# Zeudon/sound-event-localization-detection

Hardware: AMD Instinct MI355X
Metric: training clips/sec (4ch FOA 60s@24kHz) (higher is better)
Workload: dtype bf16; 1 GPU; crnn FOA 4-ch 60s clips, bs=32 windows (BASELINE configs[1]); parallelism=dp1

## Files before the change

include/seld_hip.h:

```cpp
#ifndef SELD_HIP_H_
#define SELD_HIP_H_

#include <stdint.h>

#ifdef __cplusplus
extern "C" {
#endif

int seld_init(int device);
int seld_shutdown(void);
int seld_version(void);
const char* seld_last_error(void);

int seld_set_mel_filterbank(const float* fb_host);

int seld_set_window(const float* window_host);

int seld_default_tables(float* window960, float* fb481x64, int* mel_b0_64, float* mel_wd_24x64,
                        float* mel_wu_24x64);

int64_t seld_num_frames(int64_t L);

int seld_logmel_f32(const float* pcm, int64_t N, int64_t C, int64_t L, float* out, int layout, void* stream);
int seld_logmel_i16(const int16_t* pcm, int64_t N, int64_t C, int64_t L, float* out, int layout, void* stream);
// ... 107 lines not shown
int seld_convfirst_forward(const void* in, const void* w, int w_is_bf16, int64_t w_sco, int64_t w_sci, int64_t w_sr,
                           int64_t w_ss, int64_t B, int64_t T, int64_t F, const float* bn_weight, const float* bn_bias,
                           float* running_mean, float* running_var, float momentum, float eps, void* y,
                           float* mean_invstd, float* scale_shift, float* workspace, int phases, void* stream);
int seld_convfirst_backward(const void* in, const void* w, int w_is_bf16, int64_t w_sco, int64_t w_sci, int64_t w_sr,
                            int64_t w_ss, const void* dy, int64_t B, int64_t T, int64_t F, const float* mean_invstd,
                            const float* scale_shift, void* dw, int dw_is_bf16, int64_t dw_sco, int64_t dw_sci,
                            int64_t dw_sr, int64_t dw_ss, float* dgamma, float* dbeta, float* workspace, int phases,
                            void* stream);

int64_t seld_conv_tail_workspace_floats(int C);
int seld_conv_tail_forward(const void* x, const void* residual, int is_bf16, int64_t rows, int C, int pool,
                           const float* weight, const float* bias, float* running_mean, float* running_var,
                           float momentum, float eps, int training, void* y, float* mean_invstd, float* scale_shift,
                           float* workspace, void* stream);
int seld_conv_tail_backward(const void* x, const void* residual, const void* dy, int is_bf16, int64_t rows, int C,
                            int pool, const float* mean_invstd, const float* scale_shift, void* dx, void* dresidual,
                            float* dweight, float* dbias, float* workspace, void* stream);

int seld_dwconv1d(const void* x, int is_bf16, const float* weight, const float* bias, int64_t B, int64_t T, int D, int K,
                  int flip_taps, void* y, void* stream);
int64_t seld_dwconv1d_wgrad_rows(int64_t B, int64_t T);
int seld_dwconv1d_wgrad(const void* x, const void* dy, int is_bf16, int64_t B, int64_t T, int D, int K, float* partial,
                        void* stream);

int64_t seld_gru_tile_rows(void);
int seld_gru_forward(const void* gi, int is_bf16, const void* w_hh_bf16, const float* b_hn, int64_t B,
                     int64_t T, int64_t H, void* y, void* saved_tile, void* stream);

int seld_gru_backward(const void* dy_tile, const void* saved_tile, const void* y, int is_bf16,
                      const void* w_hh_t_bf16, int64_t tiles, int64_t T, int64_t H, void* dg_tile, float* dbias,
                      void* stream);

int seld_gru_to_tile(const void* src, int elem_bytes, int64_t B, int64_t T, int ns, void* dst, void* stream);
int seld_gru_from_pair_tile(const void* dg_tile, int elem_bytes, int64_t B, int64_t T, void* dgi, void* dghn,
                            void* stream);

int seld_gru_previous_state(const void* y, int elem_bytes, int64_t B, int64_t T, void* h_prev, void* stream);

int seld_grid_decode(const void* logits, int is_bf16, int64_t w0, int64_t nw, int64_t W, int64_t total,
                     const int64_t* meta_first, const int32_t* meta_len, int64_t q0, int64_t nq, float threshold, int K,
                     int32_t* det_cell, float* det_score, int32_t* det_count, float* probs_out, void* stream);

int seld_doa_match(const int32_t* det_cell, const int32_t* det_count, int K, const int32_t* ref_offsets,
                   const int32_t* ref_dirs, int64_t nq, int I, int J, double thr_deg, int32_t* stats, double* cost,
                   void* stream);

#ifdef __cplusplus
}
#endif
#endif
```

sound-event-localization-detection_amd/csrc/gru.hip:

```cpp
#include <hip/hip_bf16.h>
#include <stdlib.h>

#include "seld_common.h"

#ifndef SELD_GRU_SEQS
#define SELD_GRU_SEQS 4
#endif

namespace seld {

constexpr int kH = 256;
constexpr int kG = 3 * kH;
constexpr int kRows = 16;
constexpr int kSeqs = SELD_GRU_SEQS;
constexpr int kParts = kRows / kSeqs;
constexpr int kU = 8 / kParts;
constexpr int kGruThreads = 512;
constexpr int kHPitch = kH + 8;
constexpr int kDghPitch = kG + 8;
constexpr int kWnBytes = 8 * 2 * 8 * 64 * 16;
static_assert(kSeqs == 8 || kSeqs == 4, "8 or 4 sequences per tile");

typedef __attribute__((ext_vector_type(8))) __bf16 bf16x8;
typedef __attribute__((ext_vector_type(4))) float f32x4;

__device__ __forceinline__ float sigmoid_f(float x) { return __builtin_amdgcn_rcpf(1.0f + __expf(-x)); }
__device__ __forceinline__ float tanh_f(float x) { return fmaf(-2.0f, __builtin_amdgcn_rcpf(1.0f + __expf(2.0f * x)), 1.0f); }

template <int kPart> __device__ __forceinline__ float shifted_part(float old, float src) {
  constexpr int ctrl = 0x110 + kPart * kSeqs;
  constexpr int banks = kSeqs == 8 ? 0xc : (1 << kPart);
  return __int_as_float(__builtin_amdgcn_update_dpp(__float_as_int(old), __float_as_int(src), ctrl, 0xf, banks, false));
}
__device__ __forceinline__ void own_values(const f32x4 (&v)[2], float (&out)[kU]) {
#pragma unroll
  for (int j = 0; j < kU; ++j) {
    float r = v[j >> 2][j & 3];
    if (kParts >= 2) r = shifted_part<1>(r, v[(kU + j) >> 2][(kU + j) & 3]);
    if (kParts == 4) {
      r = shifted_part<2>(r, v[(2 * kU + j) >> 2][(2 * kU + j) & 3]);
      r = shifted_part<3>(r, v[(3 * kU + j) >> 2][(3 * kU + j) & 3]);
    }
    out[j] = r;
  }
}

template <int kBytes> struct Raw;
template <> struct alignas(4) Raw<4> { unsigned w[1]; };
template <> struct alignas(8) Raw<8> { unsigned w[2]; };
template <> struct alignas(16) Raw<16> { unsigned w[4]; };
template <> struct alignas(16) Raw<32> { unsigned w[8]; };

typedef _Float16 f16x2 __attribute__((ext_vector_type(2)));
typedef float f32x2 __attribute__((ext_vector_type(2)));
__device__ __forceinline__ unsigned pack_bf16x2(float lo, float hi) {
  return static_cast<unsigned>(__bfloat16_as_ushort(__float2bfloat16(lo))) |
         (static_cast<unsigned>(__bfloat16_as_ushort(__float2bfloat16(hi))) << 16);
// ... 204 lines not shown
template <typename T>
__global__ __launch_bounds__(kGruThreads, 2) void gru_forward_kernel(GruFwdArgs a) {
  extern __shared__ __attribute__((aligned(16))) unsigned char smem[];
  bf16x8* wn_lds = reinterpret_cast<bf16x8*>(smem);
  __hip_bfloat16* hbuf = reinterpret_cast<__hip_bfloat16*>(smem + kWnBytes);
  const int tid = threadIdx.x;
  const int wave = tid >> 6, lane = tid & 63;
  const int q = lane >> 4, c = lane & 15;
  const __hip_bfloat16* w = a.w_hh + static_cast<long>(blockIdx.y) * kG * kH;

  bf16x8 wr[2][8], wz[2][8];
#pragma unroll
  for (int s = 0; s < 2; ++s) {
    const int unit = 32 * wave + 16 * s + c;
#pragma unroll
    for (int kk = 0; kk < 8; ++kk) {
      const int k0 = 32 * kk + 8 * q;
      wr[s][kk] = *reinterpret_cast<const bf16x8*>(w + static_cast<long>(unit) * kH + k0);
      wz[s][kk] = *reinterpret_cast<const bf16x8*>(w + static_cast<long>(kH + unit) * kH + k0);
      wn_lds[((wave * 2 + s) * 8 + kk) * 64 + lane] =
          *reinterpret_cast<const bf16x8*>(w + static_cast<long>(2 * kH + unit) * kH + k0);
    }
  }
  for (int i = tid; i < 2 * kSeqs * kHPitch; i += kGruThreads) hbuf[i] = __float2bfloat16(0.0f);
  __syncthreads();
  if (a.saved) gru_forward_steps<T, true>(a, wn_lds, hbuf, wr, wz);
  else gru_forward_steps<T, false>(a, wn_lds, hbuf, wr, wz);
}

struct GruBwdArgs {
  const void* dy;
  const void* saved;
  const void* y;
  const __hip_bfloat16* w_hh_t;
  void* dg;
  float* dbias;
  long tiles, T;
};

template <typename T> struct GruStepIn {
  PairOf<typename Types<T>::Saved> rz, ng;
  Group<typename Types<T>::Data> hp, d;
};

template <typename T>
__device__ __forceinline__ void gru_backward_steps(const GruBwdArgs& a, bf16x8* wn_lds, __hip_bfloat16* dgh,
                                                   const bf16x8 (&wrz)[2][16]) {
  typedef typename Types<T>::Data D;
  typedef typename Types<T>::Saved S;
  const int tid = threadIdx.x;
  const int wave = tid >> 6, lane = tid & 63;
  const int q = lane >> 4, c = lane & 15;
  const int seq = c % kSeqs;
  const int unit0 = lane_unit0(wave, lane);
  const int dir = blockIdx.y;
  const long tile = blockIdx.x;
  const Group<D>* dy = static_cast<const Group<D>*>(a.dy);
  const PairOf<S>* saved = static_cast<const PairOf<S>*>(a.saved);
  const T* y = static_cast<const T*>(a.y);
  PairOf<D>* dg = static_cast<PairOf<D>*>(a.dg);
  const long b = tile * kSeqs + seq;

  float dh[kU], bsum[4][kU];
#pragma unroll
  for (int i = 0; i < kU; ++i) {
    dh[i] = 0.0f;
#pragma unroll
    for (int k = 0; k < 4; ++k) bsum[k][i] = 0.0f;
  }

  auto time_of = [&](long step) { return dir == 0 ? step : a.T - 1 - step; };
  auto load_step = [&](long step, GruStepIn<T>& in) {
    const long tt = time_of(step);
    const long tprev = time_of(step > 0 ? step - 1 : 0);
    const PairOf<S>* sp = saved + tile_group(tile, a.T, tt, dir, wave, 2, 0, lane);
    in.rz = sp[0];
    in.ng = sp[64];
    in.hp = *reinterpret_cast<const Group<D>*>(y + (b * a.T + tprev) * (2 * kH) + dir * kH + unit0);
    in.d = dy[tile_group(tile, a.T, tt, dir, wave, 1, 0, lane)];
  };

  auto step = [&](long t, GruStepIn<T>& in) {
    const long tt = time_of(t);
    float r[kU], z[kU], n[kU], g[kU], hp[kU], d[kU];
    dec2<S>(in.rz, r, z);
    dec2<S>(in.ng, n, g);
    dec1<D>(in.hp, hp);
    dec1<D>(in.d, d);
    __builtin_amdgcn_sched_barrier(0);
    load_step(t > 1 ? t - 2 : 0, in);
    __builtin_amdgcn_sched_barrier(0);
    float keep[kU], da_r[kU], da_z[kU], da_n[kU], dghn[kU];
#pragma unroll
    for (int i = 0; i < kU; ++i) {
      const float hprev = t > 0 ? hp[i] : 0.0f;
      const float dtot = d[i] + dh[i];
      const float dn = dtot * (1.0f - z[i]);
      const float dz = dtot * (hprev - n[i]);
      da_n[i] = dn * (1.0f - n[i] * n[i]);
      da_z[i] = dz * z[i] * (1.0f - z[i]);
      da_r[i] = da_n[i] * g[i] * r[i] * (1.0f - r[i]);
      dghn[i] = da_n[i] * r[i];
      keep[i] = dtot * z[i];
      bsum[0][i] += da_r[i];
      bsum[1][i] += da_z[i];
      bsum[2][i] += da_n[i];
      bsum[3][i] += dghn[i];
    }
    PairOf<D>* const gp = dg + tile_group(tile, a.T, tt, dir, wave, 2, 0, lane);
    gp[0] = enc2<D>(da_r, da_z);
    gp[64] = enc2<D>(da_n, dghn);
    __hip_bfloat16* const dgh_cur = dgh + (t & 1) * (kSeqs * kDghPitch);
    __hip_bfloat16* drow = dgh_cur + seq * kDghPitch + unit0;
    *reinterpret_cast<Group<AsBF16>*>(drow) = enc1<AsBF16>(da_r);
    *reinterpret_cast<Group<AsBF16>*>(drow + kH) = enc1<AsBF16>(da_z);
    *reinterpret_cast<Group<AsBF16>*>(drow + 2 * kH) = enc1<AsBF16>(dghn);
    __syncthreads();

    f32x4 acc[2][2];
#pragma unroll
    for (int s = 0; s < 2; ++s)
#pragma unroll
      for (int i = 0; i < 4; ++i) acc[s][0][i] = acc[s][1][i] = 0.0f;
    const __hip_bfloat16* brow = dgh_cur + seq * kDghPitch + 8 * q;
    const bf16x8* wnp = wn_lds + wave * 2 * 8 * 64 + lane;
    bf16x8 d0 = *reinterpret_cast<const bf16x8*>(brow), d1 = *reinterpret_cast<const bf16x8*>(brow + 32);
#pragma unroll
    for (int kk = 0; kk < 24; ++kk) {
      bf16x8 d2 = d1;
      if (kk + 2 < 24) d2 = *reinterpret_cast<const bf16x8*>(brow + 32 * (kk + 2));
      if (kk < 16) {
        acc[0][kk & 1] = __builtin_amdgcn_mfma_f32_16x16x32_bf16(wrz[0][kk < 16 ? kk : 0], d0, acc[0][kk & 1], 0, 0, 0);
        acc[1][kk & 1] = __builtin_amdgcn_mfma_f32_16x16x32_bf16(wrz[1][kk < 16 ? kk : 0], d0, acc[1][kk & 1], 0, 0, 0);
      } else {
        const bf16x8 w0 = wnp[(kk - 16) * 64], w1 = wnp[(8 + kk - 16) * 64];
        acc[0][kk & 1] = __builtin_amdgcn_mfma_f32_16x16x32_bf16(w0, d0, acc[0][kk & 1], 0, 0, 0);
        acc[1][kk & 1] = __builtin_amdgcn_mfma_f32_16x16x32_bf16(w1, d0, acc[1][kk & 1], 0, 0, 0);
      }
      d0 = d1;
      d1 = d2;
    }
    f32x4 total[2];
#pragma unroll
    for (int s = 0; s < 2; ++s) total[s] = acc[s][0] + acc[s][1];
    float mine[kU];
    own_values(total, mine);
#pragma unroll
    for (int i = 0; i < kU; ++i) dh[i] = keep[i] + mine[i];
  };

  GruStepIn<T> in_a, in_b;
  load_step(a.T - 1, in_a);
  load_step(a.T > 1 ? a.T - 2 : 0, in_b);
  step(a.T - 1, in_a);
  long t = a.T - 2;
#pragma unroll 1
  for (; t >= 1; t -= 2) {
    step(t, in_b);
    step(t - 1, in_a);
  }
  if (t == 0) step(0, in_b);

#pragma unroll
  for (int k = 0; k < 4; ++k)
#pragma unroll
    for (int i = 0; i < kU; ++i) {
      float v = bsum[k][i];
      v += __shfl_xor(v, 1);
      v += __shfl_xor(v, 2);
      if (kSeqs == 8) v += __shfl_xor(v, 4);
      bsum[k][i] = v;
    }
  if (seq == 0) {
    float* out = a.dbias + ((tile * 2 + dir) * 4) * kH + unit0;
#pragma unroll
    for (int k = 0; k < 4; ++k)
#pragma unroll
      for (int i = 0; i < kU; ++i) out[k * kH + i] = bsum[k][i];
  }
}

template <typename T>
__global__ __launch_bounds__(kGruThreads, 2) void gru_backward_kernel(GruBwdArgs a) {
  extern __shared__ __attribute__((aligned(16))) unsigned char smem[];
  bf16x8* wn_lds = reinterpret_cast<bf16x8*>(smem);
  __hip_bfloat16* dgh = reinterpret_cast<__hip_bfloat16*>(smem + kWnBytes);
  const int tid = threadIdx.x;
  const int wave = tid >> 6, lane = tid & 63;
  const int q = lane >> 4, c = lane & 15;
  const __hip_bfloat16* wt = a.w_hh_t + static_cast<long>(blockIdx.y) * kH * kG;

  bf16x8 wrz[2][16];
#pragma unroll
  for (int s = 0; s < 2; ++s) {
    const int unit = 32 * wave + 16 * s + c;
#pragma unroll
    for (int kk = 0; kk < 16; ++kk)
      wrz[s][kk] = *reinterpret_cast<const bf16x8*>(wt + static_cast<long>(unit) * kG + 32 * kk + 8 * q);
#pragma unroll
    for (int kk = 0; kk < 8; ++kk)
      wn_lds[((wave * 2 + s) * 8 + kk) * 64 + lane] =
          *reinterpret_cast<const bf16x8*>(wt + static_cast<long>(unit) * kG + 2 * kH + 32 * kk + 8 * q);
  }
  __syncthreads();
  gru_backward_steps<T>(a, wn_lds, dgh, wrz);
}

__device__ __forceinline__ void lane_coords(int w, int lane, int& seq, int& ug) {
  seq = (lane & 15) % kSeqs;
  ug = lane_unit0(w, lane) / kU;
}

template <int kGroupBytes>
__global__ __launch_bounds__(256) void gru_to_tile_kernel(const Raw<kGroupBytes>* __restrict__ src, long B, long T,
                                                          int ns, Raw<kGroupBytes>* __restrict__ dst) {
  const long blk = blockIdx.x;
  const int dir = static_cast<int>(blk & 1);
  const long t = (blk >> 1) % T, tile = (blk >> 1) / T;
  const int groups = 8 * ns * 64;
  Raw<kGroupBytes> zero;
  __builtin_memset(&zero, 0, sizeof(zero));
  for (int g = threadIdx.x; g < groups; g += 256) {
    const int lane = g & 63, slot = (g >> 6) % ns, w = (g >> 6) / ns;
    int seq, ug;
    lane_coords(w, lane, seq, ug);
    const long b = tile * kSeqs + seq;
    Raw<kGroupBytes> v = zero;
    if (b < B) v = src[(((b * T + t) * 2 + dir) * ns + slot) * (kH / kU) + ug];
    dst[blk * groups + g] = v;
  }
}

template <int kGroupBytes>
__global__ __launch_bounds__(256) void gru_from_pair_tile_kernel(const Raw<2 * kGroupBytes>* __restrict__ src, long B,
                                                                 long T, Raw<kGroupBytes>* __restrict__ dgi,
                                                                 Raw<kGroupBytes>* __restrict__ dghn) {
  const long blk = blockIdx.x;
  const int dir = static_cast<int>(blk & 1);
// ... 102 lines not shown
  DeviceState* st = current_state();
  if (!st) return kErrNotInitialised;
  if (H != kH) return fail(kErrUnsupported, "seld_gru_forward: built for hidden size 256 (config.py:45)");
  if (B <= 0 || T <= 0) return fail(kErrInvalidArgument, "seld_gru_forward: B and T must be positive");
  if (!gi || !w_hh_bf16 || !b_hn || !y) return fail(kErrInvalidArgument, "seld_gru_forward: null pointer");
  const long tiles = (B + kSeqs - 1) / kSeqs;
  GruFwdArgs a{gi, static_cast<const __hip_bfloat16*>(w_hh_bf16), b_hn, y, saved_tile, tiles, T, B};
  const dim3 grid(static_cast<unsigned>(tiles), 2);
  const size_t lds = kWnBytes + 2 * kSeqs * kHPitch * sizeof(__hip_bfloat16);
  hipStream_t stream = static_cast<hipStream_t>(stream_);
  if (need_lds(st, kAttrGruForward)) {
    SELD_HIP_TRY(hipFuncSetAttribute(reinterpret_cast<const void*>(gru_forward_kernel<__hip_bfloat16>),
                                     hipFuncAttributeMaxDynamicSharedMemorySize, static_cast<int>(lds)));
    SELD_HIP_TRY(hipFuncSetAttribute(reinterpret_cast<const void*>(gru_forward_kernel<float>),
                                     hipFuncAttributeMaxDynamicSharedMemorySize, static_cast<int>(lds)));
    lds_attr_set(st, kAttrGruForward);
  }
  if (is_bf16) hipLaunchKernelGGL(gru_forward_kernel<__hip_bfloat16>, grid, dim3(kGruThreads), lds, stream, a);
  else hipLaunchKernelGGL(gru_forward_kernel<float>, grid, dim3(kGruThreads), lds, stream, a);
  SELD_HIP_TRY(hipGetLastError());
  return kOk;
}

int seld_gru_backward(const void* dy_tile, const void* saved_tile, const void* y, int is_bf16,
                      const void* w_hh_t_bf16, int64_t tiles, int64_t T, int64_t H, void* dg_tile, float* dbias,
                      void* stream_) {
  using namespace seld;
  DeviceState* st = current_state();
  if (!st) return kErrNotInitialised;
  if (H != kH) return fail(kErrUnsupported, "seld_gru_backward: built for hidden size 256 (config.py:45)");
  if (tiles <= 0 || T <= 0) return fail(kErrInvalidArgument, "seld_gru_backward: tiles and T must be positive");
  if (!dy_tile || !saved_tile || !y || !w_hh_t_bf16 || !dg_tile || !dbias)
    return fail(kErrInvalidArgument, "seld_gru_backward: null pointer");
  GruBwdArgs a{dy_tile, saved_tile, y, static_cast<const __hip_bfloat16*>(w_hh_t_bf16), dg_tile, dbias, tiles, T};
  const dim3 grid(static_cast<unsigned>(tiles), 2);
  const size_t lds = kWnBytes + 2 * kSeqs * kDghPitch * sizeof(__hip_bfloat16);
  hipStream_t stream = static_cast<hipStream_t>(stream_);
  if (need_lds(st, kAttrGruBackward)) {
    SELD_HIP_TRY(hipFuncSetAttribute(reinterpret_cast<const void*>(gru_backward_kernel<__hip_bfloat16>),
                                     hipFuncAttributeMaxDynamicSharedMemorySize, static_cast<int>(lds)));
    SELD_HIP_TRY(hipFuncSetAttribute(reinterpret_cast<const void*>(gru_backward_kernel<float>),
                                     hipFuncAttributeMaxDynamicSharedMemorySize, static_cast<int>(lds)));
    lds_attr_set(st, kAttrGruBackward);
  }
  if (is_bf16) hipLaunchKernelGGL(gru_backward_kernel<__hip_bfloat16>, grid, dim3(kGruThreads), lds, stream, a);
  else hipLaunchKernelGGL(gru_backward_kernel<float>, grid, dim3(kGruThreads), lds, stream, a);
  SELD_HIP_TRY(hipGetLastError());
  return kOk;
}

}
```

sound-event-localization-detection_amd/csrc/seld_common.h:

```cpp
#pragma once

#include <hip/hip_runtime.h>
#include <stdint.h>

#include <string>

#include "logmel_core.h"

namespace seld {

enum : int {
  kOk = 0,
  kErrInvalidArgument = -1,
  kErrHip = -2,
  kErrNotInitialised = -3,
  kErrUnsupported = -4,
};

void set_error(const std::string& msg);
int fail(int code, const std::string& msg);

#define SELD_HIP_TRY(expr)                                                             \
  do {                                                                                 \
    hipError_t _e = (expr);                                                            \
// ... 5 lines not shown
  bool ready = false;
  int device = -1;
  int num_cus = 0;
  float* window = nullptr;
  float* twiddle = nullptr;
  int* mel_b0 = nullptr;
  float* mel_wd = nullptr;
  float* mel_wu = nullptr;
  int* mel_pos = nullptr;
  float* mel_fb = nullptr;
  void* gcc_table = nullptr;
  hipStream_t side_stream = nullptr;
  hipEvent_t fork_event = nullptr, join_event = nullptr;
  unsigned lds_attr_done = 0;
  LogmelTables tables() const { return LogmelTables{window, twiddle, mel_b0, mel_wd, mel_wu, mel_pos}; }
};

enum LdsAttrBit : unsigned {
  kAttrGruForward = 1u << 0,
  kAttrGruBackward = 1u << 1,
  kAttrStftF32 = 1u << 2,
  kAttrStftI16 = 1u << 3,
  kAttrLogmelF32 = 1u << 4,
  kAttrLogmelI16 = 1u << 5,
  kAttrSpatial = 1u << 6,
  kAttrLogmelSpecF32 = 1u << 7,
  kAttrLogmelSpecI16 = 1u << 8,
  kAttrGccMfma = 1u << 9,
  kAttrLogmelPhasorF32 = 1u << 10,
  kAttrLogmelPhasorI16 = 1u << 11,
  kAttrGccMfmaQ15 = 1u << 12,
  kAttrLogmelIvF32 = 1u << 13,
  kAttrLogmelIvI16 = 1u << 14,
};

inline bool need_lds(const DeviceState* st, unsigned bit) { return (st->lds_attr_done & bit) == 0; }
inline void lds_attr_set(DeviceState* st, unsigned bit) { st->lds_attr_done |= bit; }

DeviceState* current_state();

int build_gcc_table(DeviceState* st);

}
```

sound-event-localization-detection_amd/seld_gru.py:

```python
import torch
import torch.nn.functional as F

import seld_native
import seld_overlap
from seld_linear import chunk_count, tall_chunks, tall_product

HIDDEN = 256


def applicable(module, x):
    low = torch.is_autocast_enabled() or x.dtype in (torch.bfloat16, torch.float16)
    if not low and not getattr(module, "allow_fp32", False):
        return False
    return (module.hidden_size == HIDDEN and module.bidirectional and module.batch_first and module.bias
            and x.dim() == 3 and x.dtype in (torch.float32, torch.bfloat16, torch.float16) and module.proj_size == 0)


class _BiGRULayer(torch.autograd.Function):
    @staticmethod
    def forward(ctx, x, w_ih, b_ih, w_hh, b_hh, overlap=False, feature_cf=None):
        ctx.overlap = overlap
        ctx.feature_cf = feature_cf
        if feature_cf is not None:
            c, f = feature_cf
# ... 4 lines not shown
            xc = x.to(cdt)
            if b_ih.dtype == torch.float32 and b_hh.dtype == torch.float32 and b_ih.is_contiguous() and b_hh.is_contiguous():
                gi_bias, b_hn = seld_native.gru_fold_bias(b_ih, b_hh.reshape(-1), cdt)
            else:
                fold = b_hh.clone()
                fold[:, 2 * HIDDEN:] = 0
                gi_bias, b_hn = (b_ih + fold.reshape(-1)).to(cdt), b_hh[:, 2 * HIDDEN:]
            gi = F.linear(xc, w_ih.to(cdt), gi_bias)
            b, t, _ = gi.shape
            need = x.requires_grad or w_ih.requires_grad or w_hh.requires_grad
            y, saved = seld_native.gru_forward(gi.view(b, t, 2, 3 * HIDDEN), w_hh, b_hn, need)
        ctx.save_for_backward(xc, w_ih, w_hh, y, saved if saved is not None else torch.empty(0))
        ctx.cdt = cdt
        ctx.dtypes = (w_ih.dtype, b_ih.dtype, w_hh.dtype, b_hh.dtype)
        return y

    @staticmethod
    def backward(ctx, dy):
        xc, w_ih, w_hh, y, saved = ctx.saved_tensors
        cdt = ctx.cdt
        b, t, _ = y.shape
        h = HIDDEN
        n = b * t
        with torch.autocast(device_type="cuda", enabled=False):
            dyc = dy.to(y.dtype)
            seld_overlap.launch_pending(dy.device)
            dgi, dghn, dbias = seld_native.gru_backward(dyc, saved, y, w_hh, raw_bias=True)
            dgi2 = dgi.view(n, 6 * h)
            x2 = xc.reshape(n, -1)
            t_wih, t_bih, t_whh, t_bhh = ctx.dtypes

            dw_ih = torch.empty((6 * h, x2.shape[1]), dtype=t_wih, device=dy.device)
            dw_hh = torch.empty((2, 3 * h, h), dtype=t_whh, device=dy.device)

            def weight_grads():
                if ctx.feature_cf is None:
                    tall_product(dgi2, x2, out=dw_ih)
                else:
                    c, f = ctx.feature_cf
                    perm = tall_product(dgi2, x2, out_dtype=t_wih)
                    dw_ih.view(6 * h, c, f).copy_(perm.view(6 * h, f, c).transpose(1, 2))
                hp = seld_native.gru_previous_state(y).view(n, 2 * h)
                chunks = chunk_count(n, 6 * h, 2 * h)
                p_gi = tall_chunks(dgi2, hp, chunks)
                p_n = tall_chunks(dghn.view(n, 2 * h), hp, chunks)
                seld_native.gru_dwhh_finish(p_gi, p_n, dw_hh)

            dx = (dgi2 @ w_ih.to(cdt)).view_as(xc)
            if ctx.overlap:
                seld_overlap.submit(dy.device, [dgi, dghn, y, xc, dw_ih, dw_hh], weight_grads)
            elif seld_overlap.conv_wgrad_side and seld_overlap.enabled and dy.is_cuda:
                seld_overlap.launch_now(dy.device, [dgi, dghn, y, xc, dw_ih, dw_hh], weight_grads, last_of_stage=True,
                                        outputs=[dw_ih, dw_hh])
            else:
                weight_grads()
            db_ih, db_hh = seld_native.gru_bias_grads(dbias)
            db_hh = db_hh.view(2, 3 * h)
        return dx.to(dy.dtype) if dx.dtype != dy.dtype and not torch.is_autocast_enabled() else dx, \
            dw_ih.view_as(dw_ih), db_ih.to(t_bih), dw_hh.view_as(dw_hh), db_hh.to(t_bhh), None, None


from seld_pack import adjacent as _adjacent, join as _join, pack as _pack


def pack_parameters(module):
    with torch.no_grad():
        for layer in range(module.num_layers):
            for kind in ("weight_ih", "bias_ih", "weight_hh", "bias_hh"):
                _pack((getattr(module, f"{kind}_l{layer}"), getattr(module, f"{kind}_l{layer}_reverse")))


def bigru_forward(module, x, feature_cf=None, overlap=False, need_hn=True):
    overlap = overlap and seld_overlap.active(x)
    params = []
    for layer in range(module.num_layers):
        p = lambda name: getattr(module, f"{name}_l{layer}")
        pr = lambda name: getattr(module, f"{name}_l{layer}_reverse")
        group = (_join(p("weight_ih"), pr("weight_ih")), _join(p("bias_ih"), pr("bias_ih")),
                 _join(p("weight_hh"), pr("weight_hh")), _join(p("bias_hh"), pr("bias_hh")))
        params.append(seld_overlap.defer(*group) if overlap and layer > 0 else group)
    out = x
    finals = []
    for layer in range(module.num_layers):
        w_ih, b_ih, w_hh, b_hh = params[layer]
        out = _BiGRULayer.apply(out, w_ih, b_ih, w_hh.view(2, 3 * HIDDEN, HIDDEN), b_hh.view(2, 3 * HIDDEN),
                                overlap and layer > 0, feature_cf if layer == 0 else None)
        if need_hn:
            finals += [out[:, -1, :HIDDEN], out[:, 0, HIDDEN:]]
        if module.training and module.dropout > 0 and layer + 1 < module.num_layers:
            out = F.dropout(out, p=module.dropout, training=True)
    return out, (torch.stack(finals, dim=0) if need_hn else None)
```

sound-event-localization-detection_amd/seld_native.py:

```python
from __future__ import annotations

import ctypes
import os
import threading
from pathlib import Path

import torch

_HERE = Path(__file__).resolve().parent
LIB_PATH = Path(os.environ["SELD_HIP_LIB"]).resolve() if os.environ.get("SELD_HIP_LIB") else _HERE / "libseld_hip.so"

N_FFT = 960
HOP = 480
N_BINS = 481
N_MELS = 64

_lock = threading.Lock()
_lib = None
_initialised_devices = set()

_i64 = ctypes.c_int64
_int = ctypes.c_int
_ptr = ctypes.c_void_p

# ... 64 lines not shown
    lib.seld_conv3x3_wgrad_workspace_floats.restype = _i64
    lib.seld_conv3x3_wgrad_workspace_floats.argtypes = [_i64, _i64, _i64, _i64, _i64]
    lib.seld_conv3x3_wgrad.argtypes = [_ptr, _ptr, _i64, _i64, _i64, _i64, _i64, _ptr, _int, _ptr, _ptr]
    lib.seld_convfirst_supported.argtypes = [_i64, _i64, _i64]
    lib.seld_convfirst_workspace_floats.restype = _i64
    lib.seld_convfirst_workspace_floats.argtypes = [_int]
    lib.seld_convfirst_forward.argtypes = [_ptr, _ptr, _int, _i64, _i64, _i64, _i64, _i64, _i64, _i64, _ptr, _ptr, _ptr, _ptr,
                                           ctypes.c_float, ctypes.c_float, _ptr, _ptr, _ptr, _ptr, _int, _ptr]
    lib.seld_convfirst_backward.argtypes = [_ptr, _ptr, _int, _i64, _i64, _i64, _i64, _ptr, _i64, _i64, _i64, _ptr, _ptr,
                                            _ptr, _int, _i64, _i64, _i64, _i64, _ptr, _ptr, _ptr, _int, _ptr]
    lib.seld_layernorm_supported.argtypes = [_i64]
    lib.seld_layernorm_workspace_floats.restype = _i64
    lib.seld_layernorm_workspace_floats.argtypes = [_i64, _i64]
    lib.seld_layernorm_forward.argtypes = [_ptr, _int, _i64, _i64, _ptr, _ptr, ctypes.c_float, _int, _ptr, _ptr, _ptr]
    lib.seld_layernorm_backward.argtypes = [_ptr, _ptr, _int, _i64, _i64, _ptr, _ptr, _ptr, _int, _ptr, _ptr, _ptr,
                                            _ptr, _ptr]
    lib.seld_conv_tail_workspace_floats.restype = _i64
    lib.seld_conv_tail_workspace_floats.argtypes = [_int]
    lib.seld_conv_tail_forward.argtypes = [_ptr, _ptr, _int, _i64, _int, _int, _ptr, _ptr, _ptr, _ptr, ctypes.c_float,
                                           ctypes.c_float, _int, _ptr, _ptr, _ptr, _ptr, _ptr]
    lib.seld_conv_tail_backward.argtypes = [_ptr, _ptr, _ptr, _int, _i64, _int, _int, _ptr, _ptr, _ptr, _ptr, _ptr, _ptr,
                                            _ptr, _ptr]
    lib.seld_dwconv1d.argtypes = [_ptr, _int, _ptr, _ptr, _i64, _i64, _int, _int, _int, _ptr, _ptr]
    lib.seld_dwconv1d_wgrad.argtypes = [_ptr, _ptr, _int, _i64, _i64, _int, _int, _ptr, _ptr]
    lib.seld_dwconv1d_wgrad_rows.argtypes = [_i64, _i64]
    lib.seld_dwconv1d_wgrad_rows.restype = ctypes.c_int64
    lib.seld_gru_to_tile.argtypes = [_ptr, _int, _i64, _i64, _int, _ptr, _ptr]
    lib.seld_gru_from_pair_tile.argtypes = [_ptr, _int, _i64, _i64, _ptr, _ptr, _ptr]
    lib.seld_gru_previous_state.argtypes = [_ptr, _int, _i64, _i64, _ptr, _ptr]
    lib.seld_gru_tile_rows.restype = _i64
    lib.seld_gru_tile_rows.argtypes = []
    lib.seld_gru_forward.argtypes = [_ptr, _int, _ptr, _ptr, _i64, _i64, _i64, _ptr, _ptr, _ptr]
    lib.seld_gru_backward.argtypes = [_ptr, _ptr, _ptr, _int, _ptr, _i64, _i64, _i64, _ptr, _ptr, _ptr]
    lib.seld_grid_decode.argtypes = [_ptr, _int, _i64, _i64, _i64, _i64, _ptr, _ptr, _i64, _i64, ctypes.c_float, _int,
                                     _ptr, _ptr, _ptr, _ptr, _ptr]
    lib.seld_doa_match.argtypes = [_ptr, _ptr, _int, _ptr, _ptr, _i64, _int, _int, ctypes.c_double, _ptr, _ptr, _ptr]
    return lib


def load_library():
    global _lib
    if _lib is not None:
        return _lib
    with _lock:
        if _lib is None:
            if not LIB_PATH.exists():
                raise SeldNativeError(
                    f"{LIB_PATH} not found: build it with `python -c 'import __graft_entry__ as g; g.build()'` "
                    f"or `make -C {_HERE / 'csrc'}`.  There is no CPU fallback.")
            lib = _declare(ctypes.CDLL(str(LIB_PATH)))
            global GRU_TILE
            GRU_TILE = int(lib.seld_gru_tile_rows())
            _lib = lib
        return _lib


def check(rc: int, what: str = "libseld_hip"):
    if rc != 0:
        msg = load_library().seld_last_error()
        raise SeldNativeError(f"{what} failed with code {rc}: {msg.decode() if msg else '?'}")


_raw_stream = getattr(torch._C, "_cuda_getCurrentRawStream", None)


def _stream_ptr(device) -> ctypes.c_void_p:
# ... 566 lines not shown

def gru_forward(gi: torch.Tensor, w_hh: torch.Tensor, b_hn: torch.Tensor, need_saved: bool):
    if not gi.is_cuda:
        raise SeldNativeError("gru_forward: tensors must live on the GPU")
    b, t, two, g3 = gi.shape
    h = g3 // 3
    if two != 2 or h != GRU_H or gi.dtype not in (torch.float32, torch.bfloat16):
        raise ValueError("gru_forward: gi must be [B, T, 2, 768] float32 or bfloat16")
    index = ensure_init(gi.device)
    gi = gi.contiguous()
    tiles = (b + GRU_TILE - 1) // GRU_TILE
    w = w_hh.to(torch.bfloat16).contiguous()
    bias = b_hn.to(torch.float32).contiguous()
    if tuple(bias.shape) != (2, h):
        raise ValueError("gru_forward: b_hn must be [2, H]")
    y = torch.empty((tiles * GRU_TILE, t, 2 * h), dtype=gi.dtype, device=gi.device)
    saved_dtype = torch.float16 if gi.dtype == torch.bfloat16 else torch.float32
    saved = torch.empty((tiles, t, 2, 8, 2, 64, 2, 8 * GRU_TILE // 16), dtype=saved_dtype, device=gi.device) \
        if need_saved else None
    with _device_guard(index):
        check(load_library().seld_gru_forward(_p(gi), int(gi.dtype == torch.bfloat16), _p(w), _p(bias), b, t,
                                              h, _p(y), _p(saved), _stream_ptr(gi.device)), "seld_gru_forward")
    return y[:b], saved


def gru_backward(dy: torch.Tensor, saved: torch.Tensor, y: torch.Tensor, w_hh: torch.Tensor, raw_bias: bool = False):
    b, t, h2 = dy.shape
    h = h2 // 2
    index = ensure_init(dy.device)
    if saved.dtype != (torch.float16 if dy.dtype == torch.bfloat16 else torch.float32):
        raise ValueError("gru_backward: saved activations do not belong to a forward pass of this dtype")
    if y.dtype != dy.dtype or tuple(y.shape) != (b, t, h2):
        raise ValueError("gru_backward: y must be the forward output matching dy")
    dy_tile = to_tile_device(dy.reshape(b, t, 2, 1, h), 1)
    tiles = dy_tile.shape[0]
    if tiles * GRU_TILE != b:
        y = torch.cat((y, y.new_zeros((tiles * GRU_TILE - b, t, h2))), dim=0)
    y = y.contiguous()
    w_t = w_hh.to(torch.bfloat16).transpose(1, 2).contiguous()
    dg_tile = torch.empty((tiles, t, 2, 8, 2, 4, 16 // GRU_TILE, GRU_TILE, 2, 8 * GRU_TILE // 16), dtype=dy.dtype,
                          device=dy.device)
    dbias = torch.empty((tiles, 2, 4, h), dtype=torch.float32, device=dy.device)
    with _device_guard(index):
        check(load_library().seld_gru_backward(_p(dy_tile), _p(saved), _p(y), int(dy.dtype == torch.bfloat16),
                                               _p(w_t), tiles, t, h, _p(dg_tile), _p(dbias), _stream_ptr(dy.device)),
              "seld_gru_backward")
    dgi, dghn = from_pair_tile_device(dg_tile, b)
    if raw_bias:
        return dgi, dghn, dbias
    return dgi, dghn, dbias.sum(dim=0) if tiles > 1 else dbias[0]



def _is_bf16(t: torch.Tensor) -> int:
    if t.dtype not in (torch.float32, torch.bfloat16):
        raise TypeError(f"float32 or bfloat16 expected, got {t.dtype}")
    return int(t.dtype == torch.bfloat16)


def gru_fold_bias(b_ih: torch.Tensor, b_hh: torch.Tensor, dtype: torch.dtype):
    if not (b_ih.is_cuda and b_ih.dtype == torch.float32 and b_hh.dtype == torch.float32 and b_ih.is_contiguous()
            and b_hh.is_contiguous() and b_ih.numel() == b_hh.numel() and b_ih.numel() % 6 == 0):
        raise SeldNativeError("gru_fold_bias: b_ih, b_hh must be contiguous fp32 GPU tensors of 2 * 3H elements")
    h = b_ih.numel() // 6
    gi_bias = torch.empty(6 * h, dtype=dtype, device=b_ih.device)
    b_hn = torch.empty((2, h), dtype=torch.float32, device=b_ih.device)
    with _device_guard(ensure_init(b_ih.device)):
        check(load_library().seld_gru_fold_bias(_p(b_ih), _p(b_hh), h, _p(gi_bias), _is_bf16(gi_bias), _p(b_hn),
                                                _stream_ptr(b_ih.device)), "seld_gru_fold_bias")
    return gi_bias, b_hn


def gru_bias_grads(partial: torch.Tensor):
    tiles, two, four, h = partial.shape
    if two != 2 or four != 4 or partial.dtype != torch.float32 or not partial.is_contiguous():
        raise SeldNativeError("gru_bias_grads: partial must be contiguous fp32 [tiles, 2, 4, H]")
    db = torch.empty((2, 6 * h), dtype=torch.float32, device=partial.device)
    with _device_guard(ensure_init(partial.device)):
        check(load_library().seld_gru_bias_grads(_p(partial), tiles, h, _p(db[0]), _p(db[1]),
                                                 _stream_ptr(partial.device)), "seld_gru_bias_grads")
    return db[0], db[1]


def sum_chunks(partial: torch.Tensor, out: torch.Tensor) -> torch.Tensor:
    if not (partial.is_cuda and partial.is_contiguous() and out.is_contiguous()
            and tuple(partial.shape[1:]) == tuple(out.shape)):
        raise SeldNativeError("sum_chunks: partial [chunks, ...] and out [...] must be contiguous with matching shapes")
    with _device_guard(ensure_init(partial.device)):
        check(load_library().seld_sum_chunks(_p(partial), _is_bf16(partial), partial.shape[0], out.numel(), _p(out),
                                             _is_bf16(out), _stream_ptr(partial.device)), "seld_sum_chunks")
    return out


def column_sums_supported(g: torch.Tensor, out: torch.Tensor) -> bool:
    return (g.is_cuda and g.dim() == 2 and g.is_contiguous() and out.is_contiguous() and g.shape[1] % 8 == 0
            and g.dtype in (torch.float32, torch.bfloat16) and out.dtype in (torch.float32, torch.bfloat16)
            and out.numel() == g.shape[1] and g.data_ptr() % 16 == 0 and g.shape[0] > 0)


def column_sums(g: torch.Tensor, out: torch.Tensor) -> torch.Tensor:
    if not column_sums_supported(g, out):
        raise SeldNativeError("column_sums: g [rows, N] contiguous bf16 / fp32 with N % 8 == 0, out [N] contiguous")
    lib = load_library()
    rows, n = g.shape
    blocks = int(lib.seld_column_sums_blocks(rows, n))
    partial = torch.empty((blocks, n), dtype=torch.float32, device=g.device)
    with _device_guard(ensure_init(g.device)):
        check(lib.seld_column_sums(_p(g), _is_bf16(g), rows, n, _p(partial), _p(out), _is_bf16(out), _stream_ptr(g.device)),
              "seld_column_sums")
    return out
# ... 227 lines not shown
```

Before: 161.4 clips/s.

## Write GRU backward gradients in row layout directly, skipping tile conversions

Adds a rows-form GRU backward kernel for bf16 with 4-sequence tiles. It reads dy and y in their natural row layout and writes dgi/dghn rows straight from the LDS staging buffer. It also loads the untransposed w_hh and transposes it in-kernel with ds_read_tr16, which removes the to_tile, from_pair_tile, cat padding and weight-transpose passes around the backward. Separately, the bias-gradient reduction moves into the overlapped weight-gradient job. The cost is one extra global store per thread each step, plus added complexity in the per-step loop.

```diff
diff --git a/include/seld_hip.h b/include/seld_hip.h
--- a/include/seld_hip.h
+++ b/include/seld_hip.h
@@ -163,6 +163,9 @@
                       const void* w_hh_t_bf16, int64_t tiles, int64_t T, int64_t H, void* dg_tile, float* dbias,
                       void* stream);
 
+int seld_gru_backward_rows(const void* dy, const void* saved_tile, const void* y, const void* w_hh_bf16, int64_t B,
+                           int64_t T, int64_t H, void* dgi, void* dghn, float* dbias, void* stream);
+
 int seld_gru_to_tile(const void* src, int elem_bytes, int64_t B, int64_t T, int ns, void* dst, void* stream);
 int seld_gru_from_pair_tile(const void* dg_tile, int elem_bytes, int64_t B, int64_t T, void* dgi, void* dghn,
                             void* stream);
diff --git a/sound-event-localization-detection_amd/csrc/gru.hip b/sound-event-localization-detection_amd/csrc/gru.hip
--- a/sound-event-localization-detection_amd/csrc/gru.hip
+++ b/sound-event-localization-detection_amd/csrc/gru.hip
@@ -18,11 +18,16 @@
 constexpr int kGruThreads = 512;
 constexpr int kHPitch = kH + 8;
 constexpr int kDghPitch = kG + 8;
+constexpr int kDgRowPitch = 4 * kH + 8;
 constexpr int kWnBytes = 8 * 2 * 8 * 64 * 16;
 static_assert(kSeqs == 8 || kSeqs == 4, "8 or 4 sequences per tile");
 
 typedef __attribute__((ext_vector_type(8))) __bf16 bf16x8;
 typedef __attribute__((ext_vector_type(4))) float f32x4;
+typedef __attribute__((ext_vector_type(4))) short s16x4;
+typedef __attribute__((ext_vector_type(8))) short s16x8;
+typedef __attribute__((address_space(3))) s16x4 lds_s16x4;
+typedef __attribute__((ext_vector_type(4))) unsigned u32x4;
 
 __device__ __forceinline__ float sigmoid_f(float x) { return __builtin_amdgcn_rcpf(1.0f + __expf(-x)); }
 __device__ __forceinline__ float tanh_f(float x) { return fmaf(-2.0f, __builtin_amdgcn_rcpf(1.0f + __expf(2.0f * x)), 1.0f); }
@@ -293,10 +298,12 @@
   const void* dy;
   const void* saved;
   const void* y;
-  const __hip_bfloat16* w_hh_t;
+  const __hip_bfloat16* w;
   void* dg;
+  void* dgi;
+  void* dghn;
   float* dbias;
-  long tiles, T;
+  long tiles, T, B;
 };
 
 template <typename T> struct GruStepIn {
@@ -304,11 +311,14 @@
   Group<typename Types<T>::Data> hp, d;
 };
 
-template <typename T>
+template <typename T, bool kRowsForm>
 __device__ __forceinline__ void gru_backward_steps(const GruBwdArgs& a, bf16x8* wn_lds, __hip_bfloat16* dgh,
                                                    const bf16x8 (&wrz)[2][16]) {
   typedef typename Types<T>::Data D;
   typedef typename Types<T>::Saved S;
+  static_assert(!kRowsForm || (sizeof(T) == 2 && kSeqs == 4), "rows form: bf16, 4 sequences per tile (LDS)");
+  constexpr int kPitch = kRowsForm ? kDgRowPitch : kDghPitch;
+  constexpr int kNSeg = kRowsForm ? 3 * kH : 2 * kH;
   const int tid = threadIdx.x;
   const int wave = tid >> 6, lane = tid & 63;
   const int q = lane >> 4, c = lane & 15;
@@ -321,6 +331,15 @@
   const T* y = static_cast<const T*>(a.y);
   PairOf<D>* dg = static_cast<PairOf<D>*>(a.dg);
   const long b = tile * kSeqs + seq;
+  const bool valid = !kRowsForm || b < a.B;
+  const long b_read = valid ? b : a.B - 1;
+  const int row_seq = tid >> 7, row_j = tid & 127;
+  const long row_b = tile * kSeqs + row_seq;
+  char* const row_out = row_j < 96
+      ? static_cast<char*>(a.dgi) + (row_b * a.T * 2 + dir) * (3 * kH * 2) + 16 * row_j
+      : static_cast<char*>(a.dghn) + (row_b * a.T * 2 + dir) * (kH * 2) + 16 * (row_j - 96);
+  const int row_step = row_j < 96 ? 2 * 3 * kH * 2 : 2 * kH * 2;
+  const unsigned lane_off = static_cast<unsigned>(((b_read * a.T * 2 + dir) * kH + unit0) * sizeof(T));
 
   float dh[kU], bsum[4][kU];
 #pragma unroll
@@ -337,8 +356,14 @@
     const PairOf<S>* sp = saved + tile_group(tile, a.T, tt, dir, wave, 2, 0, lane);
     in.rz = sp[0];
     in.ng = sp[64];
-    in.hp = *reinterpret_cast<const Group<D>*>(y + (b * a.T + tprev) * (2 * kH) + dir * kH + unit0);
-    in.d = dy[tile_group(tile, a.T, tt, dir, wave, 1, 0, lane)];
+    if (kRowsForm) {
+      in.hp = *reinterpret_cast<const Group<D>*>(reinterpret_cast<const char*>(y + tprev * (2 * kH)) + lane_off);
+      in.d = *reinterpret_cast<const Group<D>*>(reinterpret_cast<const char*>(static_cast<const T*>(a.dy) + tt * (2 * kH)) +
+                                                lane_off);
+    } else {
+      in.hp = *reinterpret_cast<const Group<D>*>(y + (b * a.T + tprev) * (2 * kH) + dir * kH + unit0);
+      in.d = dy[tile_group(tile, a.T, tt, dir, wave, 1, 0, lane)];
+    }
   };
 
   auto step = [&](long t, GruStepIn<T>& in) {
@@ -348,6 +373,10 @@
     dec2<S>(in.ng, n, g);
     dec1<D>(in.hp, hp);
     dec1<D>(in.d, d);
+    if (kRowsForm) {
+#pragma unroll
+      for (int i = 0; i < kU; ++i) d[i] = valid ? d[i] : 0.0f;
+    }
     __builtin_amdgcn_sched_barrier(0);
     load_step(t > 1 ? t - 2 : 0, in);
     __builtin_amdgcn_sched_barrier(0);
@@ -368,28 +397,35 @@
       bsum[2][i] += da_n[i];
       bsum[3][i] += dghn[i];
     }
-    PairOf<D>* const gp = dg + tile_group(tile, a.T, tt, dir, wave, 2, 0, lane);
-    gp[0] = enc2<D>(da_r, da_z);
-    gp[64] = enc2<D>(da_n, dghn);
-    __hip_bfloat16* const dgh_cur = dgh + (t & 1) * (kSeqs * kDghPitch);
-    __hip_bfloat16* drow = dgh_cur + seq * kDghPitch + unit0;
+    if (!kRowsForm) {
+      PairOf<D>* const gp = dg + tile_group(tile, a.T, tt, dir, wave, 2, 0, lane);
+      gp[0] = enc2<D>(da_r, da_z);
+      gp[64] = enc2<D>(da_n, dghn);
+    }
+    __hip_bfloat16* const dgh_cur = dgh + (t & 1) * (kSeqs * kPitch);
+    __hip_bfloat16* drow = dgh_cur + seq * kPitch + unit0;
     *reinterpret_cast<Group<AsBF16>*>(drow) = enc1<AsBF16>(da_r);
     *reinterpret_cast<Group<AsBF16>*>(drow + kH) = enc1<AsBF16>(da_z);
-    *reinterpret_cast<Group<AsBF16>*>(drow + 2 * kH) = enc1<AsBF16>(dghn);
+    if (kRowsForm) *reinterpret_cast<Group<AsBF16>*>(drow + 2 * kH) = enc1<AsBF16>(da_n);
+    *reinterpret_cast<Group<AsBF16>*>(drow + kNSeg) = enc1<AsBF16>(dghn);
     __syncthreads();
+    if (kRowsForm)
+      *reinterpret_cast<Raw<16>*>(row_out + tt * static_cast<long>(row_step)) =
+          *reinterpret_cast<const Raw<16>*>(dgh_cur + row_seq * kPitch + 8 * row_j);
 
     f32x4 acc[2][2];
 #pragma unroll
     for (int s = 0; s < 2; ++s)
 #pragma unroll
       for (int i = 0; i < 4; ++i) acc[s][0][i] = acc[s][1][i] = 0.0f;
-    const __hip_bfloat16* brow = dgh_cur + seq * kDghPitch + 8 * q;
+    const __hip_bfloat16* brow = dgh_cur + seq * kPitch + 8 * q;
     const bf16x8* wnp = wn_lds + wave * 2 * 8 * 64 + lane;
+    auto kofs = [](int kk) { return kk < 16 ? 32 * kk : kNSeg + 32 * (kk - 16); };
     bf16x8 d0 = *reinterpret_cast<const bf16x8*>(brow), d1 = *reinterpret_cast<const bf16x8*>(brow + 32);
 #pragma unroll
     for (int kk = 0; kk < 24; ++kk) {
       bf16x8 d2 = d1;
-      if (kk + 2 < 24) d2 = *reinterpret_cast<const bf16x8*>(brow + 32 * (kk + 2));
+      if (kk + 2 < 24) d2 = *reinterpret_cast<const bf16x8*>(brow + kofs(kk + 2));
       if (kk < 16) {
         acc[0][kk & 1] = __builtin_amdgcn_mfma_f32_16x16x32_bf16(wrz[0][kk < 16 ? kk : 0], d0, acc[0][kk & 1], 0, 0, 0);
         acc[1][kk & 1] = __builtin_amdgcn_mfma_f32_16x16x32_bf16(wrz[1][kk < 16 ? kk : 0], d0, acc[1][kk & 1], 0, 0, 0);
@@ -413,6 +449,11 @@
   GruStepIn<T> in_a, in_b;
   load_step(a.T - 1, in_a);
   load_step(a.T > 1 ? a.T - 2 : 0, in_b);
+  if (kRowsForm) {
+    __builtin_amdgcn_sched_barrier(0);
+    (void)*(static_cast<const volatile unsigned*>(a.saved) + tid);
+    __builtin_amdgcn_sched_barrier(0);
+  }
   step(a.T - 1, in_a);
   long t = a.T - 2;
 #pragma unroll 1
@@ -441,7 +482,7 @@
   }
 }
 
-template <typename T>
+template <typename T, bool kRowsForm>
 __global__ __launch_bounds__(kGruThreads, 2) void gru_backward_kernel(GruBwdArgs a) {
   extern __shared__ __attribute__((aligned(16))) unsigned char smem[];
   bf16x8* wn_lds = reinterpret_cast<bf16x8*>(smem);
@@ -449,22 +490,70 @@
   const int tid = threadIdx.x;
   const int wave = tid >> 6, lane = tid & 63;
   const int q = lane >> 4, c = lane & 15;
-  const __hip_bfloat16* wt = a.w_hh_t + static_cast<long>(blockIdx.y) * kH * kG;
-
   bf16x8 wrz[2][16];
-#pragma unroll
-  for (int s = 0; s < 2; ++s) {
-    const int unit = 32 * wave + 16 * s + c;
-#pragma unroll
-    for (int kk = 0; kk < 16; ++kk)
-      wrz[s][kk] = *reinterpret_cast<const bf16x8*>(wt + static_cast<long>(unit) * kG + 32 * kk + 8 * q);
-#pragma unroll
-    for (int kk = 0; kk < 8; ++kk)
-      wn_lds[((wave * 2 + s) * 8 + kk) * 64 + lane] =
-          *reinterpret_cast<const bf16x8*>(wt + static_cast<long>(unit) * kG + 2 * kH + 32 * kk + 8 * q);
+  if (kRowsForm) {
+    constexpr int kStagePitch = kH + 8;
+    static_assert(kH * kStagePitch * 2 <= kWnBytes + 2 * kSeqs * kDgRowPitch * 2, "staging image exceeds the LDS");
+    const u32x4* wg = reinterpret_cast<const u32x4*>(a.w + static_cast<long>(blockIdx.y) * kG * kH);
+    unsigned short* stage = reinterpret_cast<unsigned short*>(smem);
+    u32x4 piece[16];
+    auto fetch = [&](int gate) {
+#pragma unroll
+      for (int i = 0; i < 16; ++i) piece[i] = wg[gate * (kH * kH / 8) + i * kGruThreads + tid];
+    };
+    auto put = [&]() {
+#pragma unroll
+      for (int i = 0; i < 16; ++i)
+        *reinterpret_cast<u32x4*>(stage + (i * 16 + (tid >> 5)) * kStagePitch + (tid & 31) * 8) = piece[i];
+    };
+    const unsigned short* mine = stage + (8 * q + (c >> 2)) * kStagePitch + 32 * wave + 4 * (c & 3);
+    auto fragment = [&](int s, int kk) {
+      const unsigned short* p = mine + 32 * kk * kStagePitch + 16 * s;
+      const s16x4 lo = __builtin_amdgcn_ds_read_tr16_b64_v4i16((lds_s16x4*)p);
+      const s16x4 hi = __builtin_amdgcn_ds_read_tr16_b64_v4i16((lds_s16x4*)(p + 4 * kStagePitch));
+      const s16x8 v = __builtin_shufflevector(lo, hi, 0, 1, 2, 3, 4, 5, 6, 7);
+      return __builtin_bit_cast(bf16x8, v);
+    };
+    fetch(0);
+#pragma unroll
+    for (int gate = 0; gate < 2; ++gate) {
+      put();
+      fetch(gate + 1);
+      __syncthreads();
+#pragma unroll
+      for (int s = 0; s < 2; ++s)
+#pragma unroll
+        for (int kk = 0; kk < 8; ++kk) wrz[s][8 * gate + kk] = fragment(s, kk);
+      __syncthreads();
+    }
+    put();
+    __syncthreads();
+    bf16x8 wn[2][8];
+#pragma unroll
+    for (int s = 0; s < 2; ++s)
+#pragma unroll
+      for (int kk = 0; kk < 8; ++kk) wn[s][kk] = fragment(s, kk);
+    __syncthreads();
+#pragma unroll
+    for (int s = 0; s < 2; ++s)
+#pragma unroll
+      for (int kk = 0; kk < 8; ++kk) wn_lds[((wave * 2 + s) * 8 + kk) * 64 + lane] = wn[s][kk];
+  } else {
+    const __hip_bfloat16* wt = a.w + static_cast<long>(blockIdx.y) * kH * kG;
+#pragma unroll
+    for (int s = 0; s < 2; ++s) {
+      const int unit = 32 * wave + 16 * s + c;
+#pragma unroll
+      for (int kk = 0; kk < 16; ++kk)
+        wrz[s][kk] = *reinterpret_cast<const bf16x8*>(wt + static_cast<long>(unit) * kG + 32 * kk + 8 * q);
+#pragma unroll
+      for (int kk = 0; kk < 8; ++kk)
+        wn_lds[((wave * 2 + s) * 8 + kk) * 64 + lane] =
+            *reinterpret_cast<const bf16x8*>(wt + static_cast<long>(unit) * kG + 2 * kH + 32 * kk + 8 * q);
+    }
   }
   __syncthreads();
-  gru_backward_steps<T>(a, wn_lds, dgh, wrz);
+  gru_backward_steps<T, kRowsForm>(a, wn_lds, dgh, wrz);
 }
 
 __device__ __forceinline__ void lane_coords(int w, int lane, int& seq, int& ug) {
@@ -633,21 +722,52 @@
   if (tiles <= 0 || T <= 0) return fail(kErrInvalidArgument, "seld_gru_backward: tiles and T must be positive");
   if (!dy_tile || !saved_tile || !y || !w_hh_t_bf16 || !dg_tile || !dbias)
     return fail(kErrInvalidArgument, "seld_gru_backward: null pointer");
-  GruBwdArgs a{dy_tile, saved_tile, y, static_cast<const __hip_bfloat16*>(w_hh_t_bf16), dg_tile, dbias, tiles, T};
+  GruBwdArgs a{dy_tile, saved_tile, y, static_cast<const __hip_bfloat16*>(w_hh_t_bf16), dg_tile, nullptr, nullptr,
+               dbias, tiles, T, tiles * kSeqs};
   const dim3 grid(static_cast<unsigned>(tiles), 2);
   const size_t lds = kWnBytes + 2 * kSeqs * kDghPitch * sizeof(__hip_bfloat16);
   hipStream_t stream = static_cast<hipStream_t>(stream_);
   if (need_lds(st, kAttrGruBackward)) {
-    SELD_HIP_TRY(hipFuncSetAttribute(reinterpret_cast<const void*>(gru_backward_kernel<__hip_bfloat16>),
+    SELD_HIP_TRY(hipFuncSetAttribute(reinterpret_cast<const void*>(gru_backward_kernel<__hip_bfloat16, false>),
                                      hipFuncAttributeMaxDynamicSharedMemorySize, static_cast<int>(lds)));
-    SELD_HIP_TRY(hipFuncSetAttribute(reinterpret_cast<const void*>(gru_backward_kernel<float>),
+    SELD_HIP_TRY(hipFuncSetAttribute(reinterpret_cast<const void*>(gru_backward_kernel<float, false>),
                                      hipFuncAttributeMaxDynamicSharedMemorySize, static_cast<int>(lds)));
     lds_attr_set(st, kAttrGruBackward);
   }
-  if (is_bf16) hipLaunchKernelGGL(gru_backward_kernel<__hip_bfloat16>, grid, dim3(kGruThreads), lds, stream, a);
-  else hipLaunchKernelGGL(gru_backward_kernel<float>, grid, dim3(kGruThreads), lds, stream, a);
+  if (is_bf16) hipLaunchKernelGGL((gru_backward_kernel<__hip_bfloat16, false>), grid, dim3(kGruThreads), lds, stream, a);
+  else hipLaunchKernelGGL((gru_backward_kernel<float, false>), grid, dim3(kGruThreads), lds, stream, a);
   SELD_HIP_TRY(hipGetLastError());
   return kOk;
 }
 
-}
+int seld_gru_backward_rows(const void* dy, const void* saved_tile, const void* y, const void* w_hh_bf16, int64_t B,
+                           int64_t T, int64_t H, void* dgi, void* dghn, float* dbias, void* stream_) {
+  using namespace seld;
+  DeviceState* st = current_state();
+  if (!st) return kErrNotInitialised;
+  if (H != kH) return fail(kErrUnsupported, "seld_gru_backward_rows: built for hidden size 256 (config.py:45)");
+  if (B <= 0 || T <= 0) return fail(kErrInvalidArgument, "seld_gru_backward_rows: B and T must be positive");
+  if (!dy || !saved_tile || !y || !w_hh_bf16 || !dgi || !dghn || !dbias)
+    return fail(kErrInvalidArgument, "seld_gru_backward_rows: null pointer");
+#if SELD_GRU_SEQS == 4
+  if (B * T >= (1ll << 22))
+    return fail(kErrUnsupported, "seld_gru_backward_rows: B * T too large for 32-bit row offsets");
+  const long tiles = (B + kSeqs - 1) / kSeqs;
+  GruBwdArgs a{dy, saved_tile, y, static_cast<const __hip_bfloat16*>(w_hh_bf16), nullptr, dgi, dghn, dbias, tiles, T, B};
+  const dim3 grid(static_cast<unsigned>(tiles), 2);
+  const size_t lds = kWnBytes + 2 * kSeqs * kDgRowPitch * sizeof(__hip_bfloat16);
+  if (need_lds(st, kAttrGruBackwardRows)) {
+    SELD_HIP_TRY(hipFuncSetAttribute(reinterpret_cast<const void*>(gru_backward_kernel<__hip_bfloat16, true>),
+                                     hipFuncAttributeMaxDynamicSharedMemorySize, static_cast<int>(lds)));
+    lds_attr_set(st, kAttrGruBackwardRows);
+  }
+  hipLaunchKernelGGL((gru_backward_kernel<__hip_bfloat16, true>), grid, dim3(kGruThreads), lds,
+                     static_cast<hipStream_t>(stream_), a);
+  SELD_HIP_TRY(hipGetLastError());
+  return kOk;
+#else
+  return fail(kErrUnsupported, "seld_gru_backward_rows: needs the 4-sequence tile build (LDS)");
+#endif
+}
+
+}
diff --git a/sound-event-localization-detection_amd/csrc/seld_common.h b/sound-event-localization-detection_amd/csrc/seld_common.h
--- a/sound-event-localization-detection_amd/csrc/seld_common.h
+++ b/sound-event-localization-detection_amd/csrc/seld_common.h
@@ -61,6 +61,7 @@
   kAttrGccMfmaQ15 = 1u << 12,
   kAttrLogmelIvF32 = 1u << 13,
   kAttrLogmelIvI16 = 1u << 14,
+  kAttrGruBackwardRows = 1u << 15,
 };
 
 inline bool need_lds(const DeviceState* st, unsigned bit) { return (st->lds_attr_done & bit) == 0; }
diff --git a/sound-event-localization-detection_amd/seld_gru.py b/sound-event-localization-detection_amd/seld_gru.py
--- a/sound-event-localization-detection_amd/seld_gru.py
+++ b/sound-event-localization-detection_amd/seld_gru.py
@@ -60,8 +60,12 @@
 
             dw_ih = torch.empty((6 * h, x2.shape[1]), dtype=t_wih, device=dy.device)
             dw_hh = torch.empty((2, 3 * h, h), dtype=t_whh, device=dy.device)
+            db = torch.empty((2, 6 * h), dtype=torch.float32, device=dy.device)
+            bias_in_job = t_bih == torch.float32 and t_bhh == torch.float32
 
             def weight_grads():
+                if bias_in_job:
+                    seld_native.gru_bias_grads(dbias, out=db)
                 if ctx.feature_cf is None:
                     tall_product(dgi2, x2, out=dw_ih)
                 else:
@@ -76,16 +80,19 @@
 
             dx = (dgi2 @ w_ih.to(cdt)).view_as(xc)
             if ctx.overlap:
-                seld_overlap.submit(dy.device, [dgi, dghn, y, xc, dw_ih, dw_hh], weight_grads)
+                seld_overlap.submit(dy.device, [dgi, dghn, y, xc, dbias, dw_ih, dw_hh, db], weight_grads)
             elif seld_overlap.conv_wgrad_side and seld_overlap.enabled and dy.is_cuda:
-                seld_overlap.launch_now(dy.device, [dgi, dghn, y, xc, dw_ih, dw_hh], weight_grads, last_of_stage=True,
-                                        outputs=[dw_ih, dw_hh])
+                seld_overlap.launch_now(dy.device, [dgi, dghn, y, xc, dbias, dw_ih, dw_hh, db], weight_grads,
+                                        last_of_stage=True, outputs=[dw_ih, dw_hh, db] if bias_in_job else [dw_ih, dw_hh])
             else:
                 weight_grads()
-            db_ih, db_hh = seld_native.gru_bias_grads(dbias)
-            db_hh = db_hh.view(2, 3 * h)
+            if not bias_in_job:
+                seld_native.gru_bias_grads(dbias, out=db)
+            db_ih, db_hh = db[0], db[1].view(2, 3 * h)
+            if not bias_in_job:
+                db_ih, db_hh = db_ih.to(t_bih), db_hh.to(t_bhh)
         return dx.to(dy.dtype) if dx.dtype != dy.dtype and not torch.is_autocast_enabled() else dx, \
-            dw_ih.view_as(dw_ih), db_ih.to(t_bih), dw_hh.view_as(dw_hh), db_hh.to(t_bhh), None, None
+            dw_ih.view_as(dw_ih), db_ih, dw_hh.view_as(dw_hh), db_hh, None, None
 
 
 from seld_pack import adjacent as _adjacent, join as _join, pack as _pack
diff --git a/sound-event-localization-detection_amd/seld_native.py b/sound-event-localization-detection_amd/seld_native.py
--- a/sound-event-localization-detection_amd/seld_native.py
+++ b/sound-event-localization-detection_amd/seld_native.py
@@ -120,6 +120,7 @@
     lib.seld_gru_tile_rows.argtypes = []
     lib.seld_gru_forward.argtypes = [_ptr, _int, _ptr, _ptr, _i64, _i64, _i64, _ptr, _ptr, _ptr]
     lib.seld_gru_backward.argtypes = [_ptr, _ptr, _ptr, _int, _ptr, _i64, _i64, _i64, _ptr, _ptr, _ptr]
+    lib.seld_gru_backward_rows.argtypes = [_ptr, _ptr, _ptr, _ptr, _i64, _i64, _i64, _ptr, _ptr, _ptr, _ptr]
     lib.seld_grid_decode.argtypes = [_ptr, _int, _i64, _i64, _i64, _i64, _ptr, _ptr, _i64, _i64, ctypes.c_float, _int,
                                      _ptr, _ptr, _ptr, _ptr, _ptr]
     lib.seld_doa_match.argtypes = [_ptr, _ptr, _int, _ptr, _ptr, _i64, _int, _int, ctypes.c_double, _ptr, _ptr, _ptr]
@@ -752,6 +753,20 @@
         raise ValueError("gru_backward: saved activations do not belong to a forward pass of this dtype")
     if y.dtype != dy.dtype or tuple(y.shape) != (b, t, h2):
         raise ValueError("gru_backward: y must be the forward output matching dy")
+    if dy.dtype == torch.bfloat16 and GRU_TILE == 4:
+        tiles = (b + GRU_TILE - 1) // GRU_TILE
+        dy, y = dy.contiguous(), y.contiguous()
+        w = w_hh.to(torch.bfloat16).contiguous()
+        dgi = torch.empty((tiles * GRU_TILE, t, 2, 3, h), dtype=dy.dtype, device=dy.device)
+        dghn = torch.empty((tiles * GRU_TILE, t, 2, h), dtype=dy.dtype, device=dy.device)
+        dbias = torch.empty((tiles, 2, 4, h), dtype=torch.float32, device=dy.device)
+        with _device_guard(index):
+            check(load_library().seld_gru_backward_rows(_p(dy), _p(saved), _p(y), _p(w), b, t, h, _p(dgi), _p(dghn),
+                                                        _p(dbias), _stream_ptr(dy.device)), "seld_gru_backward_rows")
+        dgi, dghn = dgi[:b], dghn[:b]
+        if raw_bias:
+            return dgi, dghn, dbias
+        return dgi, dghn, dbias.sum(dim=0) if tiles > 1 else dbias[0]
     dy_tile = to_tile_device(dy.reshape(b, t, 2, 1, h), 1)
     tiles = dy_tile.shape[0]
     if tiles * GRU_TILE != b:
@@ -791,11 +806,14 @@
     return gi_bias, b_hn
 
 
-def gru_bias_grads(partial: torch.Tensor):
+def gru_bias_grads(partial: torch.Tensor, out: torch.Tensor = None):
     tiles, two, four, h = partial.shape
     if two != 2 or four != 4 or partial.dtype != torch.float32 or not partial.is_contiguous():
         raise SeldNativeError("gru_bias_grads: partial must be contiguous fp32 [tiles, 2, 4, H]")
-    db = torch.empty((2, 6 * h), dtype=torch.float32, device=partial.device)
+    if out is not None and not (out.dtype == torch.float32 and out.is_contiguous() and tuple(out.shape) == (2, 6 * h)
+                                and out.device == partial.device):
+        raise SeldNativeError("gru_bias_grads: out must be contiguous fp32 [2, 6H] on partial's device")
+    db = torch.empty((2, 6 * h), dtype=torch.float32, device=partial.device) if out is None else out
     with _device_guard(ensure_init(partial.device)):
         check(load_library().seld_gru_bias_grads(_p(partial), tiles, h, _p(db[0]), _p(db[1]),
                                                  _stream_ptr(partial.device)), "seld_gru_bias_grads")
```

Result: no change. 162.4 clips/s, median of 6 (+0.6%).
